# javieryu/nn_distributed_training

Hardware: NVIDIA H100
Metric: consensus node-rounds/sec (DiNNO, dist_mnist_PAPER; rounds/sec x graph nodes) (higher is better)
Workload: dtype fp64

## Files before the change

nn_distributed_training_b200/ops/csrc/common.cuh:

```cuda
#pragma once
#include <cuda_runtime.h>
#include <stdint.h>
#include <cstdlib>
#include <utility>

#define NNDT_DEVINL __device__ __forceinline__

namespace nndt {

constexpr int kWarp = 32;

NNDT_DEVINL float warp_sum(float v) {
#pragma unroll
  for (int o = 16; o > 0; o >>= 1) v += __shfl_xor_sync(0xffffffffu, v, o);
  return v;
}
NNDT_DEVINL double warp_sum(double v) {
#pragma unroll
  for (int o = 16; o > 0; o >>= 1) v += __shfl_xor_sync(0xffffffffu, v, o);
  return v;
}

NNDT_DEVINL void st_release_sys(int* p, int v) {
  asm volatile("st.release.sys.global.s32 [%0], %1;" ::"l"(p), "r"(v) : "memory");
}
NNDT_DEVINL int ld_acquire_sys(const int* p) {
  int v;
  asm volatile("ld.acquire.sys.global.s32 %0, [%1];" : "=r"(v) : "l"(p) : "memory");
  return v;
}
NNDT_DEVINL int ld_relaxed_sys(const int* p) {
  int v;
  asm volatile("ld.relaxed.sys.global.s32 %0, [%1];" : "=r"(v) : "l"(p) : "memory");
  return v;
}

NNDT_DEVINL float4 ld_stream_f4(const float* p) {
  float4 r;
  asm volatile("ld.global.L1::no_allocate.v4.f32 {%0,%1,%2,%3}, [%4];"
               : "=f"(r.x), "=f"(r.y), "=f"(r.z), "=f"(r.w)
               : "l"(p));
  return r;
}

NNDT_DEVINL void pdl_wait() { asm volatile("griddepcontrol.wait;" ::: "memory"); }
NNDT_DEVINL void pdl_launch_dependents() { asm volatile("griddepcontrol.launch_dependents;" ::: "memory"); }

template <typename... KArgs, typename... Args>
inline cudaError_t launch_pdl(void (*kernel)(KArgs...), dim3 grid, dim3 block, size_t smem, cudaStream_t st, Args&&... args) {
  cudaLaunchConfig_t cfg{};
  cfg.gridDim = grid; cfg.blockDim = block; cfg.dynamicSmemBytes = smem; cfg.stream = st;
  static const bool no_pdl = getenv("NNDT_NO_PDL") != nullptr;
  cudaLaunchAttribute attr[1];
  attr[0].id = cudaLaunchAttributeProgrammaticStreamSerialization;
  attr[0].val.programmaticStreamSerializationAllowed = 1;
  cfg.attrs = attr; cfg.numAttrs = no_pdl ? 0 : 1;
  return cudaLaunchKernelEx(&cfg, kernel, std::forward<Args>(args)...);
}

NNDT_DEVINL uint32_t smem_addr_u32(const void* p) { return (uint32_t)__cvta_generic_to_shared(p); }
NNDT_DEVINL void mbarrier_init(uint64_t* bar, uint32_t count) {
  asm volatile("mbarrier.init.shared::cta.b64 [%0], %1;" ::"r"(smem_addr_u32(bar)), "r"(count) : "memory");
  asm volatile("fence.mbarrier_init.release.cluster;" ::: "memory");
}
NNDT_DEVINL void mbarrier_expect_tx(uint64_t* bar, uint32_t bytes) {
  asm volatile("mbarrier.arrive.expect_tx.shared::cta.b64 _, [%0], %1;" ::"r"(smem_addr_u32(bar)), "r"(bytes) : "memory");
}
NNDT_DEVINL void tma_bulk_g2s(void* smem_dst, const void* gmem_src, uint32_t bytes, uint64_t* bar) {
  asm volatile("cp.async.bulk.shared::cluster.global.mbarrier::complete_tx::bytes [%0], [%1], %2, [%3];" ::"r"(
                   smem_addr_u32(smem_dst)),
               "l"(gmem_src), "r"(bytes), "r"(smem_addr_u32(bar))
               : "memory");
}
NNDT_DEVINL void mbarrier_wait_parity(uint64_t* bar, uint32_t parity) {
  const uint32_t addr = smem_addr_u32(bar);
  uint32_t done;
  do {
    asm volatile(
        "{\n\t.reg .pred p;\n\t"
        "mbarrier.try_wait.parity.shared::cta.b64 p, [%1], %2;\n\t"
        "selp.u32 %0, 1, 0, p;\n\t}\n"
        : "=r"(done)
        : "r"(addr), "r"(parity)
        : "memory");
  } while (!done);
}

NNDT_DEVINL void cluster_sync() {
  asm volatile("barrier.cluster.arrive.release.aligned;\n\tbarrier.cluster.wait.acquire.aligned;" ::: "memory");
}
NNDT_DEVINL uint32_t cluster_rank() { uint32_t r; asm volatile("mov.u32 %0, %%cluster_ctarank;" : "=r"(r)); return r; }
NNDT_DEVINL uint32_t map_to(const void* p, uint32_t rank) {
  uint32_t r;
  asm volatile("mapa.shared::cluster.u32 %0, %1, %2;" : "=r"(r) : "r"((uint32_t)__cvta_generic_to_shared(p)), "r"(rank));
  return r;
}
NNDT_DEVINL double ld_dsmem(uint32_t a) { double v; asm volatile("ld.shared::cluster.f64 %0, [%1];" : "=d"(v) : "r"(a) : "memory"); return v; }
NNDT_DEVINL void st_dsmem(uint32_t a, double v) { asm volatile("st.shared::cluster.f64 [%0], %1;" ::"r"(a), "d"(v) : "memory"); }

NNDT_DEVINL void dmma(double (&c)[4], double a0, double a1, double b) {
  asm volatile("mma.sync.aligned.m16n8k4.row.col.f64.f64.f64.f64 {%0,%1,%2,%3}, {%4,%5}, {%6}, {%0,%1,%2,%3};"
               : "+d"(c[0]), "+d"(c[1]), "+d"(c[2]), "+d"(c[3])
               : "d"(a0), "d"(a1), "d"(b));
}

template <int NJ, class FA, class FB>
NNDT_DEVINL void gemm(double (&c)[NJ][4], int m0, int n0, int K, int lane, FA A, FB B) {
  const int g = lane >> 2, t = lane & 3;
#pragma unroll 4
  for (int k0 = 0; k0 < K; k0 += 4) {
    const int k = k0 + t;
    const double a0 = A(m0 + g, k), a1 = A(m0 + g + 8, k);
#pragma unroll
    for (int j = 0; j < NJ; ++j) dmma(c[j], a0, a1, B(k, n0 + 8 * j + g));
  }
}

template <int NJ>
NNDT_DEVINL void zero(double (&c)[NJ][4]) {
#pragma unroll
  for (int j = 0; j < NJ; ++j) c[j][0] = c[j][1] = c[j][2] = c[j][3] = 0.0;
}
NNDT_DEVINL int frow(int m0, int lane, int i) { return m0 + (lane >> 2) + 8 * (i >> 1); }
NNDT_DEVINL int fcol(int n0, int lane, int i) { return n0 + 2 * (lane & 3) + (i & 1); }

template <class T> NNDT_DEVINL auto at(const T* s, int ld) { return [s, ld](int i, int j) { return s[i * ld + j]; }; }
template <class T> NNDT_DEVINL auto at_t(const T* s, int ld) { return [s, ld](int i, int j) { return s[j * ld + i]; }; }

__device__ __forceinline__ void split_tf32(float x, uint32_t& hi, uint32_t& lo) {
  asm("cvt.rna.tf32.f32 %0, %1;" : "=r"(hi) : "f"(x));
  const float r = x - __uint_as_float(hi);
  asm("cvt.rna.tf32.f32 %0, %1;" : "=r"(lo) : "f"(r));
}
__device__ __forceinline__ void mma_tf32(float (&c)[4], const uint32_t (&a)[4], const uint32_t (&b)[2]) {
  asm volatile(
      "mma.sync.aligned.m16n8k8.row.col.f32.tf32.tf32.f32 {%0,%1,%2,%3}, {%4,%5,%6,%7}, {%8,%9}, {%0,%1,%2,%3};"
      : "+f"(c[0]), "+f"(c[1]), "+f"(c[2]), "+f"(c[3])
      : "r"(a[0]), "r"(a[1]), "r"(a[2]), "r"(a[3]), "r"(b[0]), "r"(b[1]));
}
struct FragA { uint32_t hi[4], lo[4]; };
struct FragB { uint32_t hi[2], lo[2]; };
__device__ __forceinline__ FragA make_frag_a(float a0, float a1, float a2, float a3) {
  FragA f;
  split_tf32(a0, f.hi[0], f.lo[0]); split_tf32(a1, f.hi[1], f.lo[1]);
  split_tf32(a2, f.hi[2], f.lo[2]); split_tf32(a3, f.hi[3], f.lo[3]);
  return f;
}
__device__ __forceinline__ FragB make_frag_b(float b0, float b1) {
  FragB f;
  split_tf32(b0, f.hi[0], f.lo[0]); split_tf32(b1, f.hi[1], f.lo[1]);
  return f;
}
__device__ __forceinline__ void mma3(float (&c)[4], const FragA& a, const FragB& b) {
  mma_tf32(c, a.lo, b.hi);
  mma_tf32(c, a.hi, b.lo);
  mma_tf32(c, a.hi, b.hi);
}

template <int NJ, class FA, class FB>
NNDT_DEVINL void gemm(float (&c)[NJ][4], int m0, int n0, int K, int lane, FA A, FB B) {
  const int g = lane >> 2, t = lane & 3;
#pragma unroll 2
  for (int k0 = 0; k0 < K; k0 += 8) {
    const int k = k0 + t;
    const FragA a = make_frag_a(A(m0 + g, k), A(m0 + g + 8, k), A(m0 + g, k + 4), A(m0 + g + 8, k + 4));
#pragma unroll
    for (int j = 0; j < NJ; ++j) mma3(c[j], a, make_frag_b(B(k, n0 + 8 * j + g), B(k + 4, n0 + 8 * j + g)));
  }
}

NNDT_DEVINL void cp_async16(void* smem, const void* gmem) {
  uint32_t s = (uint32_t)__cvta_generic_to_shared(smem);
  asm volatile("cp.async.cg.shared.global [%0], [%1], 16;" ::"r"(s), "l"(gmem) : "memory");
}
NNDT_DEVINL void cp_async_commit() { asm volatile("cp.async.commit_group;" ::: "memory"); }
template <int N>
NNDT_DEVINL void cp_async_wait() {
  asm volatile("cp.async.wait_group %0;" ::"n"(N) : "memory");
}

}
```

nn_distributed_training_b200/ops/csrc/mnist_cl64.cu:

```cuda
#include "mnist_device.cuh"

namespace nndt {
namespace mnist {

namespace cl64 {

constexpr int NT = 640, CL = 4, CELLS = 36, KC = 108, WS = 116, HS = 68;
constexpr int PXR = 10 * HW;
constexpr int KT = (KC + 7) / 8;
constexpr int HR = 68;
NNDT_DEVINL int hr(int j) { return (j >> 4) * 17 + (j & 15); }
constexpr int PART_WC = 0, PART_BC = 75, PART_B1 = 78, PART_W2 = 142, PART_B2 = 782, PART_LOSS = 792, PART_N = 793;

template <int MS>
struct Smem {
  static constexpr int NO = MS / CL;
  static constexpr bool kDoublePix = MS <= 32;
  static constexpr int PXS = kDoublePix ? PXR + 2 : PXR;
  double w[HID * WS];
  double a[MS * WS];
  double h[MS * HS];
  alignas(16) unsigned char img[kDoublePix ? MS * PXS * 8 : MS * PXS];
  double lut[kDoublePix ? 1 : 256];
  double h_loc[NO * HR > CL * 80 ? NO * HR : CL * 80];
  double dh_loc[NO * HID];
  double part[800];
  double w2[NCLS * HR];
  alignas(16) double b1[HID];
  alignas(16) double b2[16];
  double wc[80];
  double dz[NO * 16];
  double red[NO];
  int sidx[MS];
  int label[MS];
  float valid[MS];
  unsigned char arg[MS * KC];
};
static_assert(sizeof(Smem<16>) <= 227 * 1024 && sizeof(Smem<32>) <= 227 * 1024 && sizeof(Smem<64>) <= 227 * 1024,
              "shared memory budget");

NNDT_DEVINL double wmax(double v) {
#pragma unroll
  for (int o = 16; o > 0; o >>= 1) v = fmax(v, __shfl_xor_sync(0xffffffffu, v, o));
  return v;
}
template <int H>
NNDT_DEVINL void fold_half(double (&v)[16], int lane) {
  const bool up = (lane & (2 * H)) != 0;
#pragma unroll
  for (int i = 0; i < H; ++i) {
    const double send = up ? v[i] : v[i + H], keep = up ? v[i + H] : v[i];
    v[i] = keep + __shfl_xor_sync(0xffffffffu, send, 2 * H);
  }
}
NNDT_DEVINL void warp_reduce_scatter16(double (&v)[16], int lane) {
  fold_half<8>(v, lane); fold_half<4>(v, lane); fold_half<2>(v, lane); fold_half<1>(v, lane);
  v[0] += __shfl_xor_sync(0xffffffffu, v[0], 1);
}
NNDT_DEVINL void dmma_nv(double (&c)[4], double a0, double a1, double b) {
  asm("mma.sync.aligned.m16n8k4.row.col.f64.f64.f64.f64 {%0,%1,%2,%3}, {%4,%5}, {%6}, {%0,%1,%2,%3};"
      : "+d"(c[0]), "+d"(c[1]), "+d"(c[2]), "+d"(c[3])
      : "d"(a0), "d"(a1), "d"(b));
}
template <int NJ, int K, class FA, class FB>
NNDT_DEVINL void gemm_k(double (&c)[NJ][4], int m0, int n0, int lane, FA A, FB B) {
  static_assert(K % 4 == 0, "k steps of 4");
  const int g = lane >> 2, t = lane & 3;
  double a0 = A(m0 + g, t), a1 = A(m0 + g + 8, t), b[NJ];
#pragma unroll
  for (int j = 0; j < NJ; ++j) b[j] = B(t, n0 + 8 * j + g);
#pragma unroll
  for (int k0 = 0; k0 < K; k0 += 4) {
    double na0 = 0.0, na1 = 0.0, nb[NJ];
    if (k0 + 4 < K) {
      const int k = k0 + 4 + t;
      na0 = A(m0 + g, k); na1 = A(m0 + g + 8, k);
#pragma unroll
      for (int j = 0; j < NJ; ++j) nb[j] = B(k, n0 + 8 * j + g);
    }
#pragma unroll
    for (int j = 0; j < NJ; ++j) dmma_nv(c[j], a0, a1, b[j]);
    if (k0 + 4 < K) {
      a0 = na0; a1 = na1;
#pragma unroll
      for (int j = 0; j < NJ; ++j) b[j] = nb[j];
    }
  }
}
NNDT_DEVINL void stamp(long long* prof, int idx, int tid) {
  if (prof != nullptr && tid == 0) {
    long long t;
    asm volatile("mov.u64 %0, %%globaltimer;" : "=l"(t));
    prof[idx] = t;
  }
}

template <int MS>
__global__ void __cluster_dims__(CL, 1, 1) __launch_bounds__(NT, 1)
mnist_cl64_train_kernel(const Args a, const GenericShape gs) {
  using SM = Smem<MS>;
  constexpr int NO = SM::NO, PXS = SM::PXS;
  constexpr bool kDoublePix = SM::kDoublePix;
  static_assert(MS % 16 == 0 && NO <= NT / 32, "tile geometry");
  static_assert(CELLS % 2 == 0 && NCLS % 2 == 0 && 32 + NCLS / 2 <= NT, "16-byte parameter copies");
  extern __shared__ __align__(16) unsigned char smem_raw[];
  SM& sm = *reinterpret_cast<SM*>(smem_raw);
  const int tid = threadIdx.x, warp = tid >> 5, lane = tid & 31;
  const int l = blockIdx.z, bsplit = blockIdx.y, nsplit = gridDim.y;
  const int c = (int)cluster_rank();
  const double* th = reinterpret_cast<const double*>(a.theta) + (size_t)l * a.n_pad;
  const double pmean = gs.mean, pis = gs.inv_std;
  const bool u8 = a.x_is_u8 != 0;
  double* imgd = reinterpret_cast<double*>(sm.img);
  auto pix = [&](int s, int p) -> double {
    if constexpr (kDoublePix) return imgd[s * PXS + p];
    else if (u8) return sm.lut[sm.img[s * PXR + p]];
    else return (double)__ldg(reinterpret_cast<const float*>(a.x) + (size_t)sm.sidx[s] * 784 + 6 * HW * c + p);
  };
  long long* prof = a.prof != nullptr ? a.prof + ((l * nsplit + bsplit) * CL + c) * 64 : nullptr;
  stamp(prof, 0, tid);

  const int call = a.calls != nullptr ? a.calls[l] : 0;
  const BatchGeom bg = batch_geom<true>(a, l, call);
  if (tid < MS) {
    int idx = 0, lab = 0; float ok = 0.f;
    const uint32_t t = (uint32_t)(bsplit * MS + tid);
    if (t < bg.bs) {
      ok = 1.f;
      idx = a.direct ? (int)(l * a.batch + t) : bg.shard_off + (int)feistel_permute(bg.start + t, bg.m, bg.key);
      lab = (int)a.y[idx];
    }
    sm.sidx[tid] = idx; sm.valid[tid] = ok; sm.label[tid] = lab;
  }
  if constexpr (!kDoublePix)
    if (tid < 256) sm.lut[tid] = ((double)tid * (1.0 / 255.0) - pmean) * pis;
  __syncthreads();
  constexpr int NU8 = (MS * 35 + NT - 1) / NT, NF4 = kDoublePix ? (MS * 70 + NT - 1) / NT : 1;
  uint2 pu[NU8]; float4 pf[NF4];
  if (u8) {
#pragma unroll
    for (int i = 0; i < NU8; ++i) {
      const int o = tid + i * NT;
      pu[i] = make_uint2(0, 0);
      if (o < MS * 35) {
        const int s = o / 35, q = o - s * 35;
        if (sm.valid[s] != 0.f)
          pu[i] = *reinterpret_cast<const uint2*>(reinterpret_cast<const unsigned char*>(a.x) + (size_t)sm.sidx[s] * 784 + 6 * HW * c + 8 * q);
      }
    }
  } else if constexpr (kDoublePix) {
#pragma unroll
    for (int i = 0; i < NF4; ++i) {
      const int o = tid + i * NT;
      pf[i] = make_float4(0.f, 0.f, 0.f, 0.f);
      if (o < MS * 70) {
        const int s = o / 70, q = o - s * 70;
        if (sm.valid[s] != 0.f)
          pf[i] = *reinterpret_cast<const float4*>(reinterpret_cast<const float*>(a.x) + (size_t)sm.sidx[s] * 784 + 6 * HW * c + 4 * q);
      }
    }
  }
  if (u8) {
#pragma unroll
    for (int i = 0; i < NU8; ++i) {
      const int o = tid + i * NT;
      if (o < MS * 35) {
        const int s = o / 35, q = o - s * 35;
        if constexpr (kDoublePix) {
          const uint32_t w[2] = {pu[i].x, pu[i].y};
          double* dst = imgd + s * PXS + 8 * q;
#pragma unroll
          for (int j = 0; j < 8; ++j) dst[j] = ((double)((w[j >> 2] >> (8 * (j & 3))) & 0xff) * (1.0 / 255.0) - pmean) * pis;
        } else {
          *reinterpret_cast<uint2*>(sm.img + s * PXR + 8 * q) = pu[i];
        }
      }
    }
  } else if constexpr (kDoublePix) {
#pragma unroll
    for (int i = 0; i < NF4; ++i) {
      const int o = tid + i * NT;
      if (o < MS * 70) {
        double* dst = imgd + (o / 70) * PXS + 4 * (o % 70);
        dst[0] = pf[i].x; dst[1] = pf[i].y; dst[2] = pf[i].z; dst[3] = pf[i].w;
      }
    }
  }
  stamp(prof, 1, tid);
  pdl_wait();
  pdl_launch_dependents();
  stamp(prof, 2, tid);

  constexpr int NW2 = (NCLS * HID + NT - 1) / NT;
  double wcv = 0.0, w2v[NW2];
  if (tid < 75) wcv = __ldcg(th + a.off_wc + tid);
  else if (tid < 78) wcv = __ldcg(th + a.off_bc + (tid - 75));
#pragma unroll
  for (int i = 0; i < NW2; ++i) {
    const int o = tid + i * NT;
    w2v[i] = o < NCLS * HID ? __ldcg(th + a.off_w2 + o) : 0.0;
  }
  for (int o = tid; o < HID * KC / 2; o += NT) {
    const int j = o / (KC / 2), r = o - j * (KC / 2), ch = r / (CELLS / 2), q = 2 * (r - ch * (CELLS / 2));
    cp_async16(sm.w + j * WS + ch * CELLS + q, th + a.off_w1 + (size_t)j * FC1_IN + ch * NPOOL + CELLS * c + q);
  }
  if (tid < HID / 2) cp_async16(sm.b1 + 2 * tid, th + a.off_b1 + 2 * tid);
  else if (tid >= 32 && tid < 32 + NCLS / 2) cp_async16(sm.b2 + 2 * (tid - 32), th + a.off_b2 + 2 * (tid - 32));
  cp_async_commit();
  if (tid < 78) sm.wc[tid] = wcv;
#pragma unroll
  for (int i = 0; i < NW2; ++i) {
    const int o = tid + i * NT;
    if (o < NCLS * HID) sm.w2[(o / HID) * HR + hr(o % HID)] = w2v[i];
  }
  __syncthreads();
  stamp(prof, 3, tid);

  for (int it = tid; it < MS * CELLS; it += NT) {
    const int s = it / CELLS, cell = it - s * CELLS;
    const int pr = cell / PHW, px = cell - pr * PHW;
    const int p0 = (2 * pr) * HW + 2 * px;
    auto patch_row = [&](double (&x)[6], int r) {
      if constexpr (kDoublePix) {
        const double* src = imgd + s * PXS + p0 + r * HW;
#pragma unroll
        for (int q = 0; q < 6; q += 2) {
          const double2 v = *reinterpret_cast<const double2*>(src + q);
          x[q] = v.x; x[q + 1] = v.y;
        }
      } else {
#pragma unroll
        for (int q = 0; q < 6; ++q) x[q] = pix(s, p0 + r * HW + q);
      }
    };
    double acc[F][4], x0[6], x1[6];
#pragma unroll
    for (int ch = 0; ch < F; ++ch)
#pragma unroll
      for (int i = 0; i < 4; ++i) acc[ch][i] = 0;
    patch_row(x0, 0);
#pragma unroll
    for (int ky = 0; ky < KS; ++ky) {
      patch_row(x1, ky + 1);
#pragma unroll
      for (int kx = 0; kx < KS; ++kx)
#pragma unroll
        for (int ch = 0; ch < F; ++ch) {
          const double w = sm.wc[ch * 25 + ky * 5 + kx];
          acc[ch][0] += w * x0[kx]; acc[ch][1] += w * x0[kx + 1];
          acc[ch][2] += w * x1[kx]; acc[ch][3] += w * x1[kx + 1];
        }
#pragma unroll
      for (int q = 0; q < 6; ++q) x0[q] = x1[q];
    }
    const bool ok = sm.valid[s] != 0.f;
#pragma unroll
    for (int ch = 0; ch < F; ++ch) {
      const double a00 = acc[ch][0], a01 = acc[ch][1], a10 = acc[ch][2], a11 = acc[ch][3];
      double m = a00; int ai = 0;
      if (a01 > m) { m = a01; ai = 1; }
      if (a10 > m) { m = a10; ai = 2; }
      if (a11 > m) { m = a11; ai = 3; }
      m += sm.wc[75 + ch];
      m = (ok && m > 0.0) ? m : 0.0;
      sm.a[s * WS + ch * CELLS + cell] = m;
      sm.arg[s * KC + ch * CELLS + cell] = (unsigned char)(ai | (m > 0.0 ? 4 : 0));
    }
  }
  cp_async_wait<0>();
  __syncthreads();
  stamp(prof, 4, tid);

  {
    constexpr int NJ1 = MS == 64 ? 2 : 1, NGRP = 8 / NJ1;
    if (warp < (MS / 16) * NGRP) {
      const int m0 = 16 * (warp / NGRP), n0 = 8 * NJ1 * (warp % NGRP);
      double acc[NJ1][4];
      zero(acc);
      gemm_k<NJ1, KC>(acc, m0, n0, lane, at(sm.a, WS), at_t(sm.w, WS));
#pragma unroll
      for (int j = 0; j < NJ1; ++j)
#pragma unroll
        for (int i = 0; i < 4; ++i) sm.h[frow(m0, lane, i) * HS + fcol(n0 + 8 * j, lane, i)] = acc[j][i];
    }
  }
  stamp(prof, 5, tid);
  cluster_sync();
  stamp(prof, 6, tid);
  if (c == 0 && tid == 0 && a.calls != nullptr) {
    if (a.arrive == nullptr || nsplit == 1) a.calls[l] = call + 1;
    else if (atomicAdd(a.arrive + l, 1u) == (unsigned)nsplit - 1) { a.arrive[l] = 0; a.calls[l] = call + 1; }
  }

  const int s0 = c * NO;
  const double inv_bs = 1.0 / (double)(bg.bs ? bg.bs : 1);
  if (warp < NO) {
    const int sl = warp, s = s0 + sl;
    double hv[2];
#pragma unroll
    for (int q = 0; q < 2; ++q) {
      const int j = lane + 32 * q;
      const double* src = sm.h + s * HS + j;
      double v = sm.b1[j];
#pragma unroll
      for (int r = 0; r < CL; ++r) v += ld_dsmem(map_to(src, (uint32_t)r));
      hv[q] = v > 0.0 ? v : 0.0;
      sm.h_loc[sl * HR + hr(j)] = hv[q];
    }
    __syncwarp();
    double zp[2];
#pragma unroll
    for (int r = 0; r < 2; ++r) {
      const int o = lane + 32 * r, cc = o >> 2, part = o & 3;
      double v = 0.0;
      if (o < 4 * NCLS) {
#pragma unroll
        for (int jj = 0; jj < 16; ++jj) v += sm.h_loc[sl * HR + part * 17 + jj] * sm.w2[cc * HR + part * 17 + jj];
      }
      v += __shfl_xor_sync(0xffffffffu, v, 1);
      v += __shfl_xor_sync(0xffffffffu, v, 2);
      zp[r] = v;
    }
    static_assert(NCLS > 8 && NCLS <= 16, "two rounds of four lanes per class");
    const double z0 = __shfl_sync(0xffffffffu, zp[0], (4 * lane) & 31), z1 = __shfl_sync(0xffffffffu, zp[1], (4 * lane) & 31);
    const bool cls = lane < NCLS;
    const double zc = cls ? (lane < 8 ? z0 : z1) + sm.b2[lane] : -1.0e300;
    const double mx = wmax(zc);
    const double se = warp_sum(cls ? exp(zc - mx) : 0.0);
    const double lse = mx + log(se);
    const int y = sm.label[s];
    const double ok = (double)sm.valid[s];
    const double dzc = cls ? ok * inv_bs * (exp(zc - lse) - (lane == y ? 1.0 : 0.0)) : 0.0;
    if (cls) sm.dz[sl * 16 + lane] = dzc;
    if (lane == y) sm.red[sl] = ok * (lse - zc);
    double dh[2] = {0.0, 0.0};
#pragma unroll
    for (int cc = 0; cc < NCLS; ++cc) {
      const double d = __shfl_sync(0xffffffffu, dzc, cc);
      dh[0] += d * sm.w2[cc * HR + hr(lane)];
      dh[1] += d * sm.w2[cc * HR + hr(lane + 32)];
    }
#pragma unroll
    for (int q = 0; q < 2; ++q) sm.dh_loc[sl * HID + lane + 32 * q] = hv[q] > 0.0 ? dh[q] : 0.0;
  }
  __syncthreads();
  for (int o = tid; o < NCLS * HID; o += NT) {
    const int cc = o >> 6, j = o & 63;
    double v = 0.0;
    for (int sl = 0; sl < NO; ++sl) v += sm.dz[sl * 16 + cc] * sm.h_loc[sl * HR + hr(j)];
    sm.part[PART_W2 + o] = v;
  }
  if (tid < HID) {
    double v = 0.0;
    for (int sl = 0; sl < NO; ++sl) v += sm.dh_loc[sl * HID + tid];
    sm.part[PART_B1 + tid] = v;
  } else if (tid >= 64 && tid < 64 + NCLS) {
    double v = 0.0;
    for (int sl = 0; sl < NO; ++sl) v += sm.dz[sl * 16 + (tid - 64)];
    sm.part[PART_B2 + (tid - 64)] = v;
  } else if (tid == 96) {
    double v = 0.0;
    for (int sl = 0; sl < NO; ++sl) v += sm.red[sl];
    sm.part[PART_LOSS] = v * inv_bs;
  }
  stamp(prof, 7, tid);
  cluster_sync();
  stamp(prof, 8, tid);
  auto grad_row = [&]() { return reinterpret_cast<double*>(a.grad_part) + ((size_t)l * nsplit + bsplit) * a.n_pad; };
  {
    constexpr int NE = PART_N - PART_B1, PER = (NE + CL - 1) / CL;
    const int o = PART_B1 + c * PER + tid;
    if (tid < PER && o < PART_N) {
      double* gp = grad_row();
      double v = 0.0;
#pragma unroll
      for (int r = 0; r < CL; ++r) v += ld_dsmem(map_to(sm.part + o, (uint32_t)r));
      if (o < PART_W2) gp[a.off_b1 + (o - PART_B1)] = v;
      else if (o < PART_B2) gp[a.off_w2 + (o - PART_W2)] = v;
      else if (o < PART_LOSS) gp[a.off_b2 + (o - PART_B2)] = v;
      else {
        a.loss_part[l * nsplit + bsplit] = (float)v;
        if (a.loss_mirror != nullptr) a.loss_mirror[l * nsplit + bsplit] = (float)v;
      }
    }
  }
  for (int o = tid; o < MS * HID; o += NT) {
    const int s = o >> 6, j = o & 63, r = s / NO;
    sm.h[s * HS + j] = ld_dsmem(map_to(sm.dh_loc + (s - r * NO) * HID + j, (uint32_t)r));
  }
  __syncthreads();
  stamp(prof, 9, tid);

  constexpr int NP2 = (MS / 16) * (KT / 2), NR2 = (NP2 + NT / 32 - 1) / (NT / 32);
  static_assert(KT % 2 == 0 && KC * MS + (NT / 32) * 16 <= HID * WS, "da1 and the conv-grad warp sums fit in the W slice");
  double acc2[NR2][2][4];
#pragma unroll
  for (int r = 0; r < NR2; ++r) {
    zero(acc2[r]);
    const int p = warp + r * (NT / 32);
    if (p < NP2) gemm_k<2, HID>(acc2[r], 16 * (p / (KT / 2)), 16 * (p % (KT / 2)), lane, at(sm.h, HS), at(sm.w, WS));
  }
  __syncthreads();
  stamp(prof, 10, tid);
  double* da1 = sm.w;
#pragma unroll
  for (int r = 0; r < NR2; ++r) {
    const int p = warp + r * (NT / 32);
    if (p < NP2) {
      const int m0 = 16 * (p / (KT / 2)), n0 = 16 * (p % (KT / 2));
#pragma unroll
      for (int jt = 0; jt < 2; ++jt)
#pragma unroll
        for (int i = 0; i < 4; ++i) {
          const int s = frow(m0, lane, i), k = fcol(n0 + 8 * jt, lane, i);
          if (k < KC) da1[k * MS + s] = (sm.arg[s * KC + k] & 4) ? acc2[r][jt][i] : 0.0;
        }
    }
  }
  __syncthreads();
  stamp(prof, 11, tid);
  constexpr int W3 = NT / 32 - HID / 16, NJ3 = 2;
  static_assert(KT % NJ3 == 0, "GEMM 3 passes cover the column tiles");
  if (warp >= W3) {
    double* gp = grad_row();
    const int m0 = 16 * (warp - W3);
#pragma unroll 1
    for (int n0 = 0; n0 < 8 * KT; n0 += 8 * NJ3) {
      double acc[NJ3][4];
      zero(acc);
      gemm_k<NJ3, MS>(acc, m0, n0, lane, at_t(sm.h, HS), at(sm.a, WS));
#pragma unroll
      for (int jt = 0; jt < NJ3; ++jt)
#pragma unroll
        for (int i = 0; i < 4; i += 2) {
          const int j = frow(m0, lane, i), k = fcol(n0 + 8 * jt, lane, i);
          if (k < KC) {
            const int ch = k / CELLS, cell = k - ch * CELLS;
            __stcg(reinterpret_cast<double2*>(gp + a.off_w1 + (size_t)j * FC1_IN + ch * NPOOL + CELLS * c + cell),
                   make_double2(acc[jt][i], acc[jt][i + 1]));
          }
        }
    }
    stamp(prof, 12, tid - W3 * 32);
  }
  constexpr int KW = 3, NRUN = MS * 3;
  static_assert(KS * KW < NT / 32 && F * KS <= 16, "conv-grad work split");
  double* wsums = sm.w + KC * MS;
  auto pix2 = [&](int s, int p) -> double2 {
    if constexpr (kDoublePix) return *reinterpret_cast<const double2*>(imgd + s * PXS + p);
    else return make_double2(pix(s, p), pix(s, p + 1));
  };
  if (warp < KS * KW) {
    const int ky = warp / KW;
    double acc[16];
#pragma unroll
    for (int i = 0; i < 16; ++i) acc[i] = 0.0;
#pragma unroll 1
    for (int r = tid - ky * KW * 32; r < NRUN; r += KW * 32) {
      const int s = r % MS, pr = r / MS;
      const int rb = (2 * pr + ky) * HW;
      double x0[6], x1[6];
#pragma unroll
      for (int px = 0; px < PHW; ++px) {
        const int p = rb + 2 * px;
        if (px == 0) {
#pragma unroll
          for (int q = 0; q < 6; q += 2) {
            const double2 u = pix2(s, p + q), v = pix2(s, p + HW + q);
            x0[q] = u.x; x0[q + 1] = u.y; x1[q] = v.x; x1[q + 1] = v.y;
          }
        } else {
#pragma unroll
          for (int q = 0; q < 4; ++q) { x0[q] = x0[q + 2]; x1[q] = x1[q + 2]; }
          const double2 u = pix2(s, p + 4), v = pix2(s, p + HW + 4);
          x0[4] = u.x; x0[5] = u.y; x1[4] = v.x; x1[5] = v.y;
        }
#pragma unroll
        for (int ch = 0; ch < F; ++ch) {
          const int k = ch * CELLS + pr * PHW + px;
          const double g = da1[k * MS + s];
          const int ai = sm.arg[s * KC + k] & 3;
          const double g00 = ai == 0 ? g : 0.0, g01 = ai == 1 ? g : 0.0, g10 = ai == 2 ? g : 0.0, g11 = ai == 3 ? g : 0.0;
#pragma unroll
          for (int kx = 0; kx < KS; ++kx) {
            double& t = acc[ch * KS + kx];
            t = fma(g00, x0[kx], t); t = fma(g01, x0[kx + 1], t);
            t = fma(g10, x1[kx], t); t = fma(g11, x1[kx + 1], t);
          }
        }
      }
    }
    warp_reduce_scatter16(acc, lane);
    if ((lane & 1) == 0 && (lane >> 1) < F * KS) wsums[warp * 16 + (lane >> 1)] = acc[0];
  } else if (warp == KS * KW) {
#pragma unroll 1
    for (int ch = 0; ch < F; ++ch) {
      double v = 0.0;
      for (int o = lane; o < CELLS * MS; o += 32) v += da1[ch * CELLS * MS + o];
      v = warp_sum(v);
      if (lane == 0) wsums[warp * 16 + ch] = v;
    }
  }
  __syncthreads();
  if (tid < 78) {
    double v = 0.0;
    if (tid < 75) {
      const int ch = tid / 25, t = tid - ch * 25, ky = t / KS, kx = t - ky * KS;
#pragma unroll
      for (int w = 0; w < KW; ++w) v += wsums[(ky * KW + w) * 16 + ch * KS + kx];
    } else {
      v = wsums[KS * KW * 16 + (tid - 75)];
    }
    st_dsmem(map_to(sm.h_loc + c * 80 + tid, 0u), v);
  }
  stamp(prof, 13, tid);
  cluster_sync();
  if (c == 0 && tid < 78) {
    double* gp = grad_row();
    double v = 0.0;
#pragma unroll
    for (int r = 0; r < CL; ++r) v += sm.h_loc[r * 80 + tid];
    gp[tid < 75 ? a.off_wc + tid : a.off_bc + (tid - 75)] = v;
  }
  stamp(prof, 14, tid);
}

template <int MS>
static cudaError_t prepare_ms() {
  static cudaError_t prep = cudaFuncSetAttribute(mnist_cl64_train_kernel<MS>, cudaFuncAttributeMaxDynamicSharedMemorySize, (int)sizeof(Smem<MS>));
  return prep;
}

template <int MS>
static cudaError_t launch_ms(const Args& a, const GenericShape& gs, cudaStream_t st) {
  const cudaError_t prep = prepare_ms<MS>();
  if (prep != cudaSuccess) return prep;
  cudaLaunchConfig_t cfg{};
  cfg.gridDim = dim3(CL, 64 / MS, a.L); cfg.blockDim = dim3(NT);
  cfg.dynamicSmemBytes = sizeof(Smem<MS>); cfg.stream = st;
  cudaLaunchAttribute attr[1];
  attr[0].id = cudaLaunchAttributeProgrammaticStreamSerialization;
  attr[0].val.programmaticStreamSerializationAllowed = 1;
  static const bool no_pdl = getenv("NNDT_NO_PDL") != nullptr;
  cfg.attrs = attr; cfg.numAttrs = no_pdl ? 0 : 1;
  return cudaLaunchKernelEx(&cfg, mnist_cl64_train_kernel<MS>, a, gs);
}

template <int MS>
static int max_clusters_ms() {
  if (prepare_ms<MS>() != cudaSuccess) { cudaGetLastError(); return 0; }
  cudaLaunchConfig_t cfg{};
  cfg.gridDim = dim3(CL, 1, 1); cfg.blockDim = dim3(NT); cfg.dynamicSmemBytes = sizeof(Smem<MS>);
  int n = 0;
  if (cudaOccupancyMaxActiveClusters(&n, mnist_cl64_train_kernel<MS>, &cfg) != cudaSuccess) { cudaGetLastError(); return 0; }
  return n;
}

}

cudaError_t launch_train_cl64(const Args& a, const GenericShape& gs, int nsplit, cudaStream_t st) {
  switch (nsplit) {
    case 1: return cl64::launch_ms<64>(a, gs, st);
    case 2: return cl64::launch_ms<32>(a, gs, st);
    case 4: return cl64::launch_ms<16>(a, gs, st);
  }
  return cudaErrorInvalidValue;
}

int cl64_max_active_clusters(int nsplit) {
  switch (nsplit) {
    case 1: return cl64::max_clusters_ms<64>();
    case 2: return cl64::max_clusters_ms<32>();
    case 4: return cl64::max_clusters_ms<16>();
  }
  return 0;
}

int cl64_cluster_ctas() { return cl64::CL; }

}
}
```

Measured before the change: 166,400.

## Replace cluster-wide syncs and DSMEM pulls with st.async pushes and mbarriers

For small microbatch shapes (MS<=32), the cluster CTAs no longer pull partial hidden activations, dh, and gradient shares from each other after a full cluster barrier. Each producer now pushes its values into the consumer's shared memory with st.async and completes transactions on per-buffer mbarriers, and consumers wait only on the specific barrier they need. This removes two cluster_sync round-trips and the remote-load latency from the critical path, and lets the gradient-share reduction overlap with GEMM 3. It adds shared-memory buffers and depends on the expected-transaction byte counts being exact, which risks hangs if they are wrong.

New measurement: 173,000, median of 6. 1.04x the previous value.

```diff
diff --git a/nn_distributed_training_b200/ops/csrc/common.cuh b/nn_distributed_training_b200/ops/csrc/common.cuh
--- a/nn_distributed_training_b200/ops/csrc/common.cuh
+++ b/nn_distributed_training_b200/ops/csrc/common.cuh
@@ -98,6 +98,29 @@
 NNDT_DEVINL double ld_dsmem(uint32_t a) { double v; asm volatile("ld.shared::cluster.f64 %0, [%1];" : "=d"(v) : "r"(a) : "memory"); return v; }
 NNDT_DEVINL void st_dsmem(uint32_t a, double v) { asm volatile("st.shared::cluster.f64 [%0], %1;" ::"r"(a), "d"(v) : "memory"); }
 
+NNDT_DEVINL void st_async(uint32_t a, double v, uint32_t bar) {
+  asm volatile("st.async.shared::cluster.mbarrier::complete_tx::bytes.f64 [%0], %1, [%2];" ::"r"(a), "d"(v), "r"(bar) : "memory");
+}
+NNDT_DEVINL void st_async(uint32_t a, double v0, double v1, uint32_t bar) {
+  asm volatile("st.async.shared::cluster.mbarrier::complete_tx::bytes.v2.f64 [%0], {%1, %2}, [%3];" ::"r"(a), "d"(v0), "d"(v1), "r"(bar)
+               : "memory");
+}
+NNDT_DEVINL void cluster_arrive_relaxed() { asm volatile("barrier.cluster.arrive.relaxed.aligned;" ::: "memory"); }
+NNDT_DEVINL void cluster_wait() { asm volatile("barrier.cluster.wait.acquire.aligned;" ::: "memory"); }
+NNDT_DEVINL void mbarrier_wait_parity_cluster(uint64_t* bar, uint32_t parity) {
+  const uint32_t addr = smem_addr_u32(bar);
+  uint32_t done;
+  do {
+    asm volatile(
+        "{\n\t.reg .pred p;\n\t"
+        "mbarrier.try_wait.parity.acquire.cluster.shared::cta.b64 p, [%1], %2;\n\t"
+        "selp.u32 %0, 1, 0, p;\n\t}\n"
+        : "=r"(done)
+        : "r"(addr), "r"(parity)
+        : "memory");
+  } while (!done);
+}
+
 NNDT_DEVINL void dmma(double (&c)[4], double a0, double a1, double b) {
   asm volatile("mma.sync.aligned.m16n8k4.row.col.f64.f64.f64.f64 {%0,%1,%2,%3}, {%4,%5}, {%6}, {%0,%1,%2,%3};"
                : "+d"(c[0]), "+d"(c[1]), "+d"(c[2]), "+d"(c[3])
diff --git a/nn_distributed_training_b200/ops/csrc/mnist_cl64.cu b/nn_distributed_training_b200/ops/csrc/mnist_cl64.cu
--- a/nn_distributed_training_b200/ops/csrc/mnist_cl64.cu
+++ b/nn_distributed_training_b200/ops/csrc/mnist_cl64.cu
@@ -15,11 +15,13 @@
 template <int MS>
 struct Smem {
   static constexpr int NO = MS / CL;
+  static constexpr bool kPush = MS <= 32;
+  static constexpr int PER = (PART_N - PART_B1 + CL - 1) / CL;
   static constexpr bool kDoublePix = MS <= 32;
   static constexpr int PXS = kDoublePix ? PXR + 2 : PXR;
   double w[HID * WS];
   double a[MS * WS];
-  double h[MS * HS];
+  alignas(16) double h[MS * HS];
   alignas(16) unsigned char img[kDoublePix ? MS * PXS * 8 : MS * PXS];
   double lut[kDoublePix ? 1 : 256];
   double h_loc[NO * HR > CL * 80 ? NO * HR : CL * 80];
@@ -35,6 +37,9 @@
   int label[MS];
   float valid[MS];
   unsigned char arg[MS * KC];
+  alignas(16) double hin[kPush ? CL * NO * HID : 2];
+  double shr[kPush ? CL * PER : 1];
+  uint64_t bar[3];
 };
 static_assert(sizeof(Smem<16>) <= 227 * 1024 && sizeof(Smem<32>) <= 227 * 1024 && sizeof(Smem<64>) <= 227 * 1024,
               "shared memory budget");
@@ -119,6 +124,18 @@
   };
   long long* prof = a.prof != nullptr ? a.prof + ((l * nsplit + bsplit) * CL + c) * 64 : nullptr;
   stamp(prof, 0, tid);
+  constexpr bool kPush = SM::kPush;
+  constexpr int PER = SM::PER;
+  if constexpr (kPush) {
+    static_assert(CL * NO * HID >= CL * 80, "rank 0's partial-H buffer holds the conv-gradient shares");
+    if (tid == 0) {
+      for (int i = 0; i < 3; ++i) mbarrier_init(&sm.bar[i], 1);
+      mbarrier_expect_tx(&sm.bar[0], CL * NO * HID * 8);
+      mbarrier_expect_tx(&sm.bar[1], MS * HID * 8);
+      mbarrier_expect_tx(&sm.bar[2], CL * min(PER, PART_N - PART_B1 - c * PER) * 8);
+    }
+    cluster_arrive_relaxed();
+  }
 
   const int call = a.calls != nullptr ? a.calls[l] : 0;
   const BatchGeom bg = batch_geom<true>(a, l, call);
@@ -273,11 +290,24 @@
 
   {
     constexpr int NJ1 = MS == 64 ? 2 : 1, NGRP = 8 / NJ1;
-    if (warp < (MS / 16) * NGRP) {
-      const int m0 = 16 * (warp / NGRP), n0 = 8 * NJ1 * (warp % NGRP);
-      double acc[NJ1][4];
-      zero(acc);
-      gemm_k<NJ1, KC>(acc, m0, n0, lane, at(sm.a, WS), at_t(sm.w, WS));
+    const bool busy = warp < (MS / 16) * NGRP;
+    const int m0 = 16 * (warp / NGRP), n0 = 8 * NJ1 * (warp % NGRP);
+    double acc[NJ1][4];
+    zero(acc);
+    if (busy) gemm_k<NJ1, KC>(acc, m0, n0, lane, at(sm.a, WS), at_t(sm.w, WS));
+    if constexpr (kPush) {
+      cluster_wait();
+      if (busy) {
+#pragma unroll
+        for (int j = 0; j < NJ1; ++j)
+#pragma unroll
+          for (int i = 0; i < 4; i += 2) {
+            const int s = frow(m0, lane, i), r = s / NO;
+            st_async(map_to(sm.hin + (c * NO + s - r * NO) * HID + fcol(n0 + 8 * j, lane, i), (uint32_t)r), acc[j][i],
+                     acc[j][i + 1], map_to(&sm.bar[0], (uint32_t)r));
+          }
+      }
+    } else if (busy) {
 #pragma unroll
       for (int j = 0; j < NJ1; ++j)
 #pragma unroll
@@ -285,7 +315,11 @@
     }
   }
   stamp(prof, 5, tid);
-  cluster_sync();
+  if constexpr (kPush) {
+    if (warp < NO) mbarrier_wait_parity_cluster(&sm.bar[0], 0);
+  } else {
+    cluster_sync();
+  }
   stamp(prof, 6, tid);
   if (c == 0 && tid == 0 && a.calls != nullptr) {
     if (a.arrive == nullptr || nsplit == 1) a.calls[l] = call + 1;
@@ -303,7 +337,10 @@
       const double* src = sm.h + s * HS + j;
       double v = sm.b1[j];
 #pragma unroll
-      for (int r = 0; r < CL; ++r) v += ld_dsmem(map_to(src, (uint32_t)r));
+      for (int r = 0; r < CL; ++r) {
+        if constexpr (kPush) v += sm.hin[(r * NO + sl) * HID + j];
+        else v += ld_dsmem(map_to(src, (uint32_t)r));
+      }
       hv[q] = v > 0.0 ? v : 0.0;
       sm.h_loc[sl * HR + hr(j)] = hv[q];
     }
@@ -341,54 +378,79 @@
       dh[1] += d * sm.w2[cc * HR + hr(lane + 32)];
     }
 #pragma unroll
-    for (int q = 0; q < 2; ++q) sm.dh_loc[sl * HID + lane + 32 * q] = hv[q] > 0.0 ? dh[q] : 0.0;
+    for (int q = 0; q < 2; ++q) {
+      dh[q] = hv[q] > 0.0 ? dh[q] : 0.0;
+      sm.dh_loc[sl * HID + lane + 32 * q] = dh[q];
+    }
+    if constexpr (kPush) {
+      const int e = (2 * lane) & 31;
+      const double e0 = __shfl_sync(0xffffffffu, dh[0], e), e1 = __shfl_sync(0xffffffffu, dh[1], e);
+      const double o0 = __shfl_sync(0xffffffffu, dh[0], e + 1), o1 = __shfl_sync(0xffffffffu, dh[1], e + 1);
+#pragma unroll
+      for (int r = 0; r < CL; ++r)
+        st_async(map_to(sm.h + s * HS + 2 * lane, (uint32_t)r), lane < 16 ? e0 : e1, lane < 16 ? o0 : o1,
+                 map_to(&sm.bar[1], (uint32_t)r));
+    }
   }
   __syncthreads();
+  auto share = [&](int o, double v) {
+    if constexpr (kPush) {
+      const int e = o - PART_B1, q = e / PER;
+      st_async(map_to(sm.shr + c * PER + (e - q * PER), (uint32_t)q), v, map_to(&sm.bar[2], (uint32_t)q));
+    } else {
+      sm.part[o] = v;
+    }
+  };
   for (int o = tid; o < NCLS * HID; o += NT) {
     const int cc = o >> 6, j = o & 63;
     double v = 0.0;
     for (int sl = 0; sl < NO; ++sl) v += sm.dz[sl * 16 + cc] * sm.h_loc[sl * HR + hr(j)];
-    sm.part[PART_W2 + o] = v;
+    share(PART_W2 + o, v);
   }
   if (tid < HID) {
     double v = 0.0;
     for (int sl = 0; sl < NO; ++sl) v += sm.dh_loc[sl * HID + tid];
-    sm.part[PART_B1 + tid] = v;
+    share(PART_B1 + tid, v);
   } else if (tid >= 64 && tid < 64 + NCLS) {
     double v = 0.0;
     for (int sl = 0; sl < NO; ++sl) v += sm.dz[sl * 16 + (tid - 64)];
-    sm.part[PART_B2 + (tid - 64)] = v;
+    share(PART_B2 + (tid - 64), v);
   } else if (tid == 96) {
     double v = 0.0;
     for (int sl = 0; sl < NO; ++sl) v += sm.red[sl];
-    sm.part[PART_LOSS] = v * inv_bs;
+    share(PART_LOSS, v * inv_bs);
   }
   stamp(prof, 7, tid);
-  cluster_sync();
+  if constexpr (kPush) mbarrier_wait_parity_cluster(&sm.bar[1], 0);
+  else cluster_sync();
   stamp(prof, 8, tid);
   auto grad_row = [&]() { return reinterpret_cast<double*>(a.grad_part) + ((size_t)l * nsplit + bsplit) * a.n_pad; };
-  {
-    constexpr int NE = PART_N - PART_B1, PER = (NE + CL - 1) / CL;
-    const int o = PART_B1 + c * PER + tid;
-    if (tid < PER && o < PART_N) {
-      double* gp = grad_row();
-      double v = 0.0;
-#pragma unroll
-      for (int r = 0; r < CL; ++r) v += ld_dsmem(map_to(sm.part + o, (uint32_t)r));
-      if (o < PART_W2) gp[a.off_b1 + (o - PART_B1)] = v;
-      else if (o < PART_B2) gp[a.off_w2 + (o - PART_W2)] = v;
-      else if (o < PART_LOSS) gp[a.off_b2 + (o - PART_B2)] = v;
-      else {
-        a.loss_part[l * nsplit + bsplit] = (float)v;
-        if (a.loss_mirror != nullptr) a.loss_mirror[l * nsplit + bsplit] = (float)v;
-      }
-    }
-  }
-  for (int o = tid; o < MS * HID; o += NT) {
-    const int s = o >> 6, j = o & 63, r = s / NO;
-    sm.h[s * HS + j] = ld_dsmem(map_to(sm.dh_loc + (s - r * NO) * HID + j, (uint32_t)r));
-  }
-  __syncthreads();
+  auto reduce_share = [&](int i) {
+    const int o = PART_B1 + c * PER + i;
+    if (o >= PART_N) return;
+    double* gp = grad_row();
+    double v = 0.0;
+#pragma unroll
+    for (int r = 0; r < CL; ++r) {
+      if constexpr (kPush) v += sm.shr[r * PER + i];
+      else v += ld_dsmem(map_to(sm.part + o, (uint32_t)r));
+    }
+    if (o < PART_W2) gp[a.off_b1 + (o - PART_B1)] = v;
+    else if (o < PART_B2) gp[a.off_w2 + (o - PART_W2)] = v;
+    else if (o < PART_LOSS) gp[a.off_b2 + (o - PART_B2)] = v;
+    else {
+      a.loss_part[l * nsplit + bsplit] = (float)v;
+      if (a.loss_mirror != nullptr) a.loss_mirror[l * nsplit + bsplit] = (float)v;
+    }
+  };
+  if constexpr (!kPush) {
+    if (tid < PER) reduce_share(tid);
+    for (int o = tid; o < MS * HID; o += NT) {
+      const int s = o >> 6, j = o & 63, r = s / NO;
+      sm.h[s * HS + j] = ld_dsmem(map_to(sm.dh_loc + (s - r * NO) * HID + j, (uint32_t)r));
+    }
+    __syncthreads();
+  }
   stamp(prof, 9, tid);
 
   constexpr int NP2 = (MS / 16) * (KT / 2), NR2 = (NP2 + NT / 32 - 1) / (NT / 32);
@@ -422,6 +484,10 @@
   constexpr int W3 = NT / 32 - HID / 16, NJ3 = 2;
   static_assert(KT % NJ3 == 0, "GEMM 3 passes cover the column tiles");
   if (warp >= W3) {
+    if constexpr (kPush) {
+      mbarrier_wait_parity_cluster(&sm.bar[2], 0);
+      for (int i = tid - W3 * 32; i < PER; i += NT - W3 * 32) reduce_share(i);
+    }
     double* gp = grad_row();
     const int m0 = 16 * (warp - W3);
 #pragma unroll 1
@@ -502,6 +568,7 @@
     }
   }
   __syncthreads();
+  double* cin = kPush ? sm.hin : sm.h_loc;
   if (tid < 78) {
     double v = 0.0;
     if (tid < 75) {
@@ -511,7 +578,7 @@
     } else {
       v = wsums[KS * KW * 16 + (tid - 75)];
     }
-    st_dsmem(map_to(sm.h_loc + c * 80 + tid, 0u), v);
+    st_dsmem(map_to(cin + c * 80 + tid, 0u), v);
   }
   stamp(prof, 13, tid);
   cluster_sync();
@@ -519,7 +586,7 @@
     double* gp = grad_row();
     double v = 0.0;
 #pragma unroll
-    for (int r = 0; r < CL; ++r) v += sm.h_loc[r * 80 + tid];
+    for (int r = 0; r < CL; ++r) v += cin[r * 80 + tid];
     gp[tid < 75 ? a.off_wc + tid : a.off_bc + (tid - 75)] = v;
   }
   stamp(prof, 14, tid);
```
